# dcvan24/pivot-scheduling

Measured on AMD Instinct MI355X. Metric: task x host placement candidates scored/sec (HBM GB/s % peak) at 1/2/4/8 MI355X, higher is better.
Workload: dtype f64; 1 GPU; synthetic 1000000 hosts x 10000 ready tasks per round, 20 zones, cost_aware best-fit, one independent scenario per GPU; scenarios_per_gpu=1, tasks_per_round=10000, zones=20, policy=ca_bf, parallelism=scenario-sharded x1 (no data-path collective)

## Files before the change

pivot-scheduling_amd/csrc/pvt_zwalk.hip:

```cpp
#include <hip/hip_runtime.h>
#include <stdint.h>

#include "pivot_place.h"
#include "pvt_device.h"
#include "pvt_kernels.h"
#include "pvt_zwin_dev.h"

namespace pvt {

constexpr int ZW_THREADS = 256;
constexpr int ZW_WAVES = ZW_THREADS / 64;
constexpr int ZW_SCAN = 8;
constexpr int ZW_MINB = ZW_MIN_PARTS;
constexpr int ZW_PR = 8;
constexpr double ZW_BIG = 0x1p500;

#ifndef PVT_ZW_UNROLL
#define PVT_ZW_UNROLL 8
#endif
#ifndef PVT_ZW_CF
#define PVT_ZW_CF 0
#endif
constexpr int ZW_UNROLL = PVT_ZW_UNROLL;
constexpr int ZW_SB = 64;
template <int WM>
struct ZwalkLDS {
  double wa[4][WM];
  int32_t wid[WM];
  int32_t wz[WM];
  uint64_t zm[WM / 64];
  double csum[ZMAX * ZMAX], bsum[ZMAX * ZMAX];
  int32_t cnt[ZW_SCAN][ZW_WAVES];
  double red[ZW_WAVES][12];
  double smin[ZW_SB][4];
  double lg[128][4];
  int32_t lgid[128];
  int32_t rwho[64], rstart[64];
  uint64_t sbits[CHAIN_MAX / 64];
  uint32_t amask[ZMAX];
  uint32_t umask;
  int32_t nwin, bail;
  int32_t touch[WM / 64];
};

__device__ __forceinline__ double nan_max(double a, double b) {
  return (a != a || b <= a) ? a : b;
}
__device__ __forceinline__ double wave_nmax_d(double v) {
  return wave_reduce_d(v, [](double a, double b) { return nan_max(a, b); });
}

__global__ __launch_bounds__(256) void host_min_kernel(const double* avail, int H, int lo, int hi,
                                                       double* part) {
  __shared__ double red[4][4];
  const int tid = threadIdx.x, lane = tid & 63, wave = tid >> 6;
  double m[4] = {DINF, DINF, DINF, DINF};
  for (int h = lo + blockIdx.x * 256 + tid; h < hi; h += gridDim.x * 256)
#pragma unroll
    for (int r = 0; r < 4; r++) m[r] = fmin(m[r], avail[(size_t)r * H + h]);
#pragma unroll
  for (int r = 0; r < 4; r++) {
    m[r] = wave_min_d(m[r]);
    if (lane == 0) red[wave][r] = m[r];
  }
  __syncthreads();
  if (tid < 4) {
    double v = red[0][tid];
    for (int w = 1; w < 4; w++) v = fmin(v, red[w][tid]);
    part[blockIdx.x * 4 + tid] = v;
  }
}

template <int N> struct IntC { static constexpr int value = N; };

constexpr int ZW_CAP = 128;
__device__ __forceinline__ int lowbit_exp(double v) {
  const uint64_t b = (uint64_t)__double_as_longlong(v);
  const uint64_t m = b & ((1ull << 52) - 1);
  const int e = (int)((b >> 52) & 0x7ff);
  if (e == 0) return m ? -1074 + __builtin_ctzll(m) : 4096;
  return (e - 1075) + __builtin_ctzll(m | (1ull << 52));
}
__device__ __forceinline__ int high_exp(double v) {
  return (int)(((uint64_t)__double_as_longlong(v) >> 52) & 0x7ff) - 1023;
}
template <bool STRICT>
__device__ __forceinline__ int copies_cf(double x, double d, bool& sure) {
  if (__double_as_longlong(d) == 0) return ZW_CAP;
  const double q = x * __builtin_amdgcn_rcp(d);
  double kf = STRICT ? __builtin_ceil(q) - 1.0 : __builtin_floor(q);
  kf = __builtin_fmin(kf, (double)ZW_CAP);
  const double e0 = __builtin_fma(-kf, d, x), e1 = __builtin_fma(-(kf + 1.0), d, x);
  const double big = __builtin_fabs(x) + (kf + 1.0) * d;
  const bool nice = high_exp(big) + 2 <= min(lowbit_exp(x), lowbit_exp(d)) + 53;
  const double err = nice ? 0.0 : (kf + 2.0) * 0x1p-52 * (big + d);
  const bool fit0 = STRICT ? (e0 > err) : (e0 >= err && (nice || e0 > err));
  const bool out1 = kf >= (double)ZW_CAP || (STRICT ? (e1 <= -err && (nice || e1 < -err)) : (e1 < -err));
  sure = sure && kf >= 1.0 && fit0 && out1 && (q == q);
  return (int)kf;
}

#define UNI(c) (__builtin_amdgcn_readfirstlane((int)(c)) != 0)

template <bool STRICT>
__device__ __forceinline__ bool fit_res(double m) { return STRICT ? (m > 0.0) : (m >= 0.0); }

__device__ __forceinline__ void wave_lds_sync() {
  __atomic_signal_fence(__ATOMIC_SEQ_CST);
  __builtin_amdgcn_s_waitcnt(0xc07f);
  __atomic_signal_fence(__ATOMIC_SEQ_CST);
}

template <int WM = ZW_M>
__device__ __forceinline__ void compact_zone_window(const int32_t* zone, int Z, uint32_t U,
                                                    int h_lo, int h_hi, int32_t* wid, int32_t* wz,
                                                    int32_t (*cnt)[ZW_WAVES], int32_t* nwin) {
  compact_zone_window_t<WM, ZW_THREADS, ZW_SCAN>(zone, Z, U, h_lo, h_hi, wid, wz, cnt, nwin);
}

#ifdef PVT_STAMPS
__device__ __forceinline__ uint64_t zstamp() {
  uint64_t t;
  __builtin_amdgcn_sched_barrier(0);
  asm volatile("s_memtime %0\n\ts_waitcnt lgkmcnt(0)" : "=s"(t)::"memory");
  __builtin_amdgcn_sched_barrier(0);
  return t;
}
#endif

template <bool KEYED, bool STRICT, bool FF = false, int WM = ZW_M, bool FAST = false>
__global__ __launch_bounds__(ZW_THREADS) void zwalk_kernel(ZwalkArgs A) {
  static_assert(!FF || (!KEYED && STRICT), "FF: chain mode, strict fit");
  static_assert(WM == ZW_M || !KEYED, "keyed / ordered / sharded windows: ZW_M hosts");
  __shared__ ZwalkLDS<WM> S;
#ifdef PVT_STAMPS
  const uint64_t t_start = zstamp();
  uint64_t n_chunks = 0, n_switch = 0, n_bulk = 0, n_runs = 0;
  uint64_t st_search = 0, st_p1 = 0, st_p2 = 0, n_probe = 0, n_iter = 0, st_batch = 0, n_single = 0;
  uint64_t st_setup = 0, st_loop = 0, st_who = 0, st_rep = 0;
  uint64_t n_cf = 0;
#endif
  const int b = blockIdx.x, tid = threadIdx.x, lane = tid & 63, wave = tid >> 6;
  const bool tabm = !KEYED && A.tab.nch > 0;
  const int base = KEYED ? 0 : tabm ? A.tab.coff[b] : A.coff[b];
  const int nt = KEYED ? A.knt : tabm ? A.tab.coff[b + 1] - A.tab.coff[b] : A.coff[b + 1] - base;
  const int32_t* gcmap = KEYED ? nullptr : A.cmap + base;
  auto cmap_at = [&](int i) -> int { return gcmap[i]; };
  const bool segm = !KEYED && (tabm || A.cseg);
  int32_t* status = A.status + 2 * b;
  const int Z = A.Z, H = A.H;
  auto report = [&](int s0, int s1) {
    status[0] = s0; status[1] = s1;
    if (!KEYED && A.hstat) { A.hstat[2 * b] = s0; A.hstat[2 * b + 1] = s1; }
  };

  auto publish_map = [&]() {
    if (tabm) {
      int32_t* wmap = const_cast<int32_t*>(A.cmap) + base;
      for (int k = A.tab.csoff[b]; k < A.tab.csoff[b + 1]; k++) {
        const int sg = A.tab.csegid[k], c0 = A.tab.seg_cstart[sg], o0 = A.tab.seg_off[sg];
        const int len = A.tab.seg_off[sg + 1] - o0;
        for (int i = tid; i < len; i += ZW_THREADS) wmap[c0 + i] = o0 + i;
      }
      if (b == 0) {
        const int ns = A.tab.nseg, nc = A.tab.nch;
        for (int i = tid; i <= ns; i += ZW_THREADS) {
          A.tab.o_seg_off[i] = A.tab.seg_off[i];
          if (i < ns) { A.tab.o_seg_chain[i] = A.tab.seg_chain[i]; A.tab.o_seg_cstart[i] = A.tab.seg_cstart[i]; }
        }
        for (int i = tid; i <= nc; i += ZW_THREADS) A.tab.o_coff[i] = A.tab.coff[i];
      }
    }
  };
  double mn[4];
  uint32_t U;
  int nwin;
#ifdef PVT_STAMPS
  uint64_t t_load, t_cert, t_win, t_cap;
#endif
  if constexpr (FAST) {
    static_assert(!KEYED && !FF && WM == ZW_M && ZW_M == 4 * ZW_THREADS, "fast prologue: best-fit chains");
    static_assert(ZW_ENT <= 64 && ZW_ENT <= ZW_SB, "entries: a lane each, in rwho / rstart / lg");
    const int j = min((int)A.cert.cwin[b], ZMAX - 1);
    const ZoneWindow* const zw = &A.zpre->w[j];
    const int ZZ = Z * Z;
    double cs[4], bs[4], ha[4];
#pragma unroll
    for (int u = 0; u < 4; u++) {
      const int i = tid + u * ZW_THREADS;
      cs[u] = i < ZZ ? A.csum[i] : 0.0;
      bs[u] = i < ZZ ? A.bsum[i] : 0.0;
    }
#pragma unroll
    for (int r = 0; r < 4; r++) ha[r] = A.hmin[tid * 4 + r];
    const uint32_t zu = A.zpre->U[j];
    const int zn = zw->n, zbad = zw->bad;
    int32_t wi[4], wzv[4];
    double wv[4][4];
#pragma unroll
    for (int u = 0; u < 4; u++) {
      const int p = tid + u * ZW_THREADS;
      wi[u] = zw->id[p];
      wzv[u] = zw->z[p];
#pragma unroll
      for (int r = 0; r < 4; r++) wv[u][r] = zw->a[r][p];
    }
    const int k0 = A.tab.csoff[b], k1 = A.tab.csoff[b + 1];
    double mxv = -DINF;
    bool badv = false;
    for (int k = k0 + wave; k < k1; k += ZW_WAVES) {
      const int sg = A.tab.csegid[k], c0 = A.tab.seg_cstart[sg];
      const int len = A.tab.seg_off[sg + 1] - A.tab.seg_off[sg];
      const GroupCert* const gc = A.cert.rec + min((int)A.cert.seg_grp[sg], GCOMPACT_MAX - 1);
      const int ne = (len + 63) >> 6, e = A.cert.seg_ent[sg] + lane;
      const bool on = lane < ne && lane < GC_SUB && e < ZW_ENT;
      double sm[4];
#pragma unroll
      for (int r = 0; r < 4; r++) sm[r] = on ? gc->smin[lane][r] : DINF;
      const double gm = lane < 4 ? gc->mx[lane] : -DINF;
      badv |= gc->bad != 0 || gc->n != len;
      mxv = fmax(mxv, gm);
      if (on) {
#pragma unroll
        for (int r = 0; r < 4; r++) S.lg[e][r] = sm[r];
        S.rstart[e] = c0 + 64 * lane;
        S.rwho[e] = c0 + min(64 * lane + 64, len);
      }
    }
    publish_map();
#pragma unroll
    for (int u = 0; u < 4; u++) {
      const int i = tid + u * ZW_THREADS;
      if (i < ZZ) { S.csum[i] = cs[u]; S.bsum[i] = bs[u]; }
    }
    if (tid < CHAIN_MAX / 64) S.sbits[tid] = 0;
    if (tid < WM / 64) S.touch[tid] = 0;
    if (tid < ZW_SB) {
#pragma unroll
      for (int r = 0; r < 4; r++) S.smin[tid][r] = -DINF;
    }
    nwin = min(zn, ZW_M);
#pragma unroll
    for (int u = 0; u < 4; u++) {
      const int p = tid + u * ZW_THREADS;
      if (p < nwin) {
        S.wid[p] = wi[u];
        S.wz[p] = wzv[u];
#pragma unroll
        for (int r = 0; r < 4; r++) S.wa[r][p] = wv[u][r];
      }
    }
#pragma unroll
    for (int r = 0; r < 4; r++) ha[r] = wave_min_d(ha[r]);
    const bool wbadv = __ballot(badv) != 0;
    if (lane < 4) S.red[wave][lane] = mxv;
    if (lane == 0) {
#pragma unroll
      for (int r = 0; r < 4; r++) S.red[wave][8 + r] = ha[r];
      S.cnt[0][wave] = wbadv ? 1 : 0;
    }
#ifdef PVT_STAMPS
    t_load = zstamp();
#endif
    __syncthreads();
    if (tid < Z) {
      uint32_t m = 0;
      for (int z = 0; z < Z; z++) m |= (S.csum[tid * Z + z] == 0.0) ? (1u << z) : 0u;
      S.amask[tid] = m;
    }
    for (int k = k0 + tid; k < k1; k += ZW_THREADS) {
      const int p = A.tab.seg_cstart[A.tab.csegid[k]];
      if (p > 0 && p < CHAIN_MAX) atomicOr(&S.sbits[p >> 6], 1ull << (p & 63));
    }
    double mx[4];
    bool bad = false;
#pragma unroll
    for (int w = 0; w < ZW_WAVES; w++) bad |= S.cnt[0][w] != 0;
#pragma unroll
    for (int r = 0; r < 4; r++) {
      mx[r] = fmax(fmax(S.red[0][r], S.red[1][r]), fmax(S.red[2][r], S.red[3][r]));
      ha[r] = fmin(fmin(S.red[0][8 + r], S.red[1][8 + r]), fmin(S.red[2][8 + r], S.red[3][8 + r]));
    }
    const int ne = min((int)A.cert.cent[b], ZW_ENT);
    {
      double v = lane < ne ? S.lg[lane][wave] : DINF;
#pragma unroll
      for (int off = 1; off < 64; off <<= 1) v = fmin(v, __shfl_down(v, off));
      if (lane < ne) {
        const int q = (S.rstart[lane] + 63) >> 6;
        if (q * 64 < S.rwho[lane] && q < ZW_SB) S.smin[q][wave] = v;
      }
      if (lane == 0) S.red[0][4 + wave] = v;
    }
    bool sep = false;
#pragma unroll
    for (int r = 0; r < 4; r++) sep |= (ha[r] - mx[r] >= 0x1p-288);
    U = zu;
    const bool cover = zu != 0 && (A.cert.cu[b] & ~zu) == 0;
    const bool stop = bad || !sep || nt <= 0 || nt > CHAIN_MAX || !cover || zbad != 0 || nwin <= 0;
#ifdef PVT_STAMPS
    t_cert = t_win = t_cap = zstamp();
#endif
    __syncthreads();
    if (tid == 0) {
      int cert = stop ? 0 : ZW_CERT_FAST;
#pragma unroll
      for (int r = 0; r < 4; r++) {
        const double mnr = S.red[0][4 + r];
        cert |= ((mx[r] <= 0.0 && mnr >= 0.0) ? (1 << r) : 0) | ((ha[r] >= 0x1p-287) ? (16 << r) : 0);
      }
      if (A.hcert) A.hcert[b] = cert;
      if (stop) report(0, nt <= 0 ? 0 : 1);
    }
    if (A.cmax && tid < 4) A.cmax[b * 4 + tid] = mx[tid];
    if (stop) return;
  } else {
    static_assert(ZMAX * ZMAX <= 4 * ZW_THREADS && ZW_MINB == ZW_THREADS, "prologue loads");
    const int ZZ = KEYED ? 0 : Z * Z;
    double cs[4], bs[4];
#pragma unroll
    for (int u = 0; u < 4; u++) {
      const int i = tid + u * ZW_THREADS;
      cs[u] = i < ZZ ? A.csum[i] : 0.0;
      bs[u] = i < ZZ ? A.bsum[i] : 0.0;
    }
    double ha[4] = {FF ? -DINF : DINF, FF ? -DINF : DINF, FF ? -DINF : DINF, FF ? -DINF : DINF};
    if (!KEYED) {
#pragma unroll
      for (int r = 0; r < 4; r++) {
        const double x = A.hmin[tid * 4 + r];
        ha[r] = FF ? nan_max(ha[r], x) : fmin(ha[r], x);
      }
    }
    publish_map();
    int wv[ZW_PR];
    if (tabm) {
      const int k0 = A.tab.csoff[b], k1 = A.tab.csoff[b + 1];
#pragma unroll
      for (int u = 0; u < ZW_PR; u++) {
        const int i = u * ZW_THREADS + tid;
        int v = -1;
        for (int k = k0; k < k1; k++) {
          const int sg = A.tab.csegid[k], c0 = A.tab.seg_cstart[sg];
          if (i >= c0) v = A.tab.seg_off[sg] + (i - c0);
        }
        wv[u] = i < nt ? v : -1;
      }
    } else {
#pragma unroll
      for (int u = 0; u < ZW_PR; u++) {
        const int i = u * ZW_THREADS + tid;
        wv[u] = i < nt ? (KEYED ? i : gcmap[i]) : -1;
      }
    }
    const int sg0 = tabm ? A.tab.csoff[b] : (!KEYED && A.cseg) ? A.csoff[b] : 0;
    const int sg1 = tabm ? A.tab.csoff[b + 1] : (!KEYED && A.cseg) ? A.csoff[b + 1] : 0;
    const uint32_t zpu = (!KEYED && WM == ZW_M && A.zpre && lane < Z) ? A.zpre->U[lane] : 0u;

#pragma unroll
    for (int u = 0; u < 4; u++) {
      const int i = tid + u * ZW_THREADS;
      if (i < ZZ) { S.csum[i] = cs[u]; S.bsum[i] = bs[u]; }
    }
    if (tid == 0) { S.umask = 0; S.nwin = 0; S.bail = 0; }
    if (tid < CHAIN_MAX / 64) S.sbits[tid] = 0;
    if (tid < WM / 64) S.touch[tid] = 0;
#ifdef PVT_STAMPS
    t_load = zstamp();
#endif
    __syncthreads();
    if (!KEYED && tid < Z) {
      uint32_t m = 0;
      for (int z = 0; z < Z; z++) m |= (S.csum[tid * Z + z] == 0.0) ? (1u << z) : 0u;
      S.amask[tid] = m;
    }
    if (tabm) {
      for (int k = sg0 + tid; k < sg1; k += ZW_THREADS) {
        const int p = A.tab.seg_cstart[A.tab.csegid[k]];
        if (p > 0 && p < CHAIN_MAX) atomicOr(&S.sbits[p >> 6], 1ull << (p & 63));
      }
    } else {
      for (int k = sg0 + tid; k < sg1; k += ZW_THREADS) {
        const int p = A.cseg[k];
        if (p > 0 && p < CHAIN_MAX) atomicOr(&S.sbits[p >> 6], 1ull << (p & 63));
      }
    }

    uint32_t abits = 0;
    double mx[4] = {-DINF, -DINF, -DINF, -DINF};
    mn[0] = mn[1] = mn[2] = mn[3] = DINF;
    bool bad = false;
    for (int i0 = 0; i0 < nt; i0 += ZW_PR * ZW_THREADS) {
      int av[ZW_PR], wn[ZW_PR];
      double dv[ZW_PR][4];
#pragma unroll
      for (int u = 0; u < ZW_PR; u++) {
        const int w = max(wv[u], 0);
        av[u] = A.anc[w];
#pragma unroll
        for (int r = 0; r < 4; r++) dv[u][r] = A.dem[(size_t)w * 4 + r];
      }
#pragma unroll
      for (int u = 0; u < ZW_PR; u++) {
        const int i = i0 + ZW_PR * ZW_THREADS + u * ZW_THREADS + tid;
        wn[u] = i < nt ? (KEYED ? i : cmap_at(i)) : -1;
      }
#pragma unroll
      for (int u = 0; u < ZW_PR; u++) {
        const bool ok = wv[u] >= 0;
        double bm[4];
#pragma unroll
        for (int r = 0; r < 4; r++) bm[r] = ok ? dv[u][r] : DINF;
        if (ok) {
          const int a = av[u];
          if (a < 0 || a >= Z) {
            bad = true;
          } else {
            abits |= 1u << a;
#pragma unroll
            for (int r = 0; r < 4; r++) {
              bad |= !(__builtin_fabs(dv[u][r]) <= ZW_BIG);
              mx[r] = fmax(mx[r], dv[u][r]);
              mn[r] = fmin(mn[r], dv[u][r]);
            }
          }
        }
        const int blk = (i0 + u * ZW_THREADS) / 64 + wave;
        if (blk < ZW_SB - 1 && blk * 64 < nt) {
#pragma unroll
          for (int r = 0; r < 4; r++) bm[r] = wave_min_d(bm[r]);
          if (lane == 0) {
#pragma unroll
            for (int r = 0; r < 4; r++) S.smin[blk][r] = bm[r];
          }
        }
      }
#pragma unroll
      for (int u = 0; u < ZW_PR; u++) wv[u] = wn[u];
    }
    __syncthreads();
    uint32_t um = 0;
    if (!KEYED)
      for (uint32_t m = abits; m; m &= m - 1) um |= S.amask[__builtin_ctz(m)];
#pragma unroll
    for (int r = 0; r < 4; r++) {
      mx[r] = wave_max_d(mx[r]);
      mn[r] = wave_min_d(mn[r]);
      ha[r] = FF ? wave_nmax_d(ha[r]) : wave_min_d(ha[r]);
    }
    if (lane == 0) {
#pragma unroll
      for (int r = 0; r < 4; r++) { S.red[wave][r] = mx[r]; S.red[wave][4 + r] = mn[r]; S.red[wave][8 + r] = ha[r]; }
    }
    if (bad) S.bail = 1;
    if (um) atomicOr(&S.umask, um);
    __syncthreads();
#ifdef PVT_STAMPS
    t_cert = zstamp();
#endif
#pragma unroll
    for (int r = 0; r < 4; r++) {
      for (int w = 1; w < ZW_WAVES; w++) {
        mx[r] = fmax(mx[r], S.red[w][r]);
        mn[r] = fmin(mn[r], S.red[w][4 + r]);
        ha[r] = FF ? nan_max(ha[r], S.red[w][8 + r]) : fmin(ha[r], S.red[w][8 + r]);
      }
      mx[r] = fmax(mx[r], S.red[0][r]);
      mn[r] = fmin(mn[r], S.red[0][4 + r]);
      ha[r] = FF ? nan_max(ha[r], S.red[0][8 + r]) : fmin(ha[r], S.red[0][8 + r]);
    }
    if (!KEYED && A.cmax && tid < 4) A.cmax[b * 4 + tid] = mx[tid];
    if (!KEYED && A.hcert && tid == 0) {
      int cert = 0;
      if (!FF) {
#pragma unroll
        for (int r = 0; r < 4; r++)
          cert |= ((mx[r] <= 0.0 && mn[r] >= 0.0) ? (1 << r) : 0) | ((ha[r] >= 0x1p-287) ? (16 << r) : 0);
      }
      A.hcert[b] = cert;
    }
    bool sep = KEYED;
    if (FF) {
      sep = true;
#pragma unroll
      for (int r = 0; r < 4; r++) sep &= (ha[r] <= 0x1p298) && (mn[r] >= 0.0);
    } else {
#pragma unroll
      for (int r = 0; r < 4; r++) sep |= (ha[r] - mx[r] >= 0x1p-288);
    }
    U = S.umask;
    if (S.bail || !sep || nt <= 0 || (!KEYED && nt > CHAIN_MAX)) {
      if (tid == 0) report(0, (KEYED || nt <= 0) ? 0 : 1);
      return;
    }
    const FrontierSlot* pw = A.pwin ? A.pwin + (KEYED ? 0 : b) : nullptr;
    const ZoneWindow* zw = nullptr;
    if (!KEYED && WM == ZW_M && !pw && A.zpre && U != 0) {
      const uint64_t cover = __ballot(zpu != 0 && (U & ~zpu) == 0);
      if (cover) {
        const int j = __builtin_ctzll(cover);
        zw = &A.zpre->w[j];
        U = (uint32_t)__builtin_amdgcn_readlane((int)zpu, j);
      }
    }
    if (pw) {
      const int nw = min(pw->n, ZW_M);
      for (int p = tid; p < nw; p += ZW_THREADS) {
        const int32_t h = pw->id[p];
        S.wid[p] = h;
        S.wz[p] = KEYED ? 0 : A.zone[h];
      }
      if (tid == 0) S.nwin = nw;
      __syncthreads();
    } else if (zw) {
      const int nw = min(zw->n, ZW_M);
      for (int p = tid; p < nw; p += ZW_THREADS) { S.wid[p] = zw->id[p]; S.wz[p] = zw->z[p]; }
      if (tid == 0) S.nwin = nw;
      __syncthreads();
    } else if (KEYED) {
      const int nw = min(A.kn_dev ? *A.kn_dev : A.kn, ZW_M);
      for (int p = tid; p < nw; p += ZW_THREADS) { S.wid[p] = A.lo + A.kperm[p]; S.wz[p] = 0; }
      if (tid == 0) S.nwin = nw;
      __syncthreads();
    } else {
      compact_zone_window<WM>(A.zone, Z, U, 0, H, S.wid, S.wz, S.cnt, &S.nwin);
    }
    nwin = S.nwin;
#ifdef PVT_STAMPS
    t_win = zstamp();
#endif
    bool wbad = false;
    ZwUndo* const ud = (!KEYED && A.undo) ? A.undo + b : nullptr;
    if (ud && tid == 0) ud->count = nwin;
    static_assert(WM <= ZW_MBIG, "ZwUndo holds every window");
    static_assert(WM % (4 * ZW_THREADS) == 0, "window capacities: four hosts per thread per pass");
    for (int p0 = 0; p0 < WM && p0 < nwin; p0 += 4 * ZW_THREADS) {
      double v[4][4];
#pragma unroll
      for (int u = 0; u < 4; u++) {
        const int p = p0 + u * ZW_THREADS + tid;
        const int h = p < nwin ? S.wid[p] : 0;
#pragma unroll
        for (int r = 0; r < 4; r++)
          v[u][r] = p >= nwin ? 0.0 : (pw ? pw->a[r][p] : zw ? zw->a[r][p] : A.avail[(size_t)r * H + h]);
      }
#pragma unroll
      for (int u = 0; u < 4; u++) {
        const int p = p0 + u * ZW_THREADS + tid;
        if (p < nwin) {
#pragma unroll
          for (int r = 0; r < 4; r++) {
            wbad |= !(__builtin_fabs(v[u][r]) <= ZW_BIG);
            S.wa[r][p] = v[u][r];
          }
          if (ud) {
            ud->id[p] = S.wid[p];
#pragma unroll
            for (int r = 0; r < 4; r++) ud->a[r][p] = v[u][r];
          }
        }
      }
    }
    if (wbad) S.bail = 1;
    __syncthreads();
#ifdef PVT_STAMPS
    t_cap = zstamp();
#endif
    if (S.bail || nwin == 0) {
      if (tid == 0) report(0, KEYED ? 0 : 1);
      return;
    }
    const int nsb = min((nt + 63) >> 6, ZW_SB);
    for (int blk = ZW_SB - 1 + wave; blk < nsb; blk += ZW_WAVES) {
      const int i1 = blk == ZW_SB - 1 ? nt : min(nt, blk * 64 + 64);
      double bm[4] = {DINF, DINF, DINF, DINF};
      for (int i = blk * 64 + lane; i < i1; i += 64) {
        const int w = KEYED ? i : cmap_at(i);
#pragma unroll
        for (int r = 0; r < 4; r++) bm[r] = fmin(bm[r], A.dem[(size_t)w * 4 + r]);
      }
#pragma unroll
      for (int r = 0; r < 4; r++) bm[r] = wave_min_d(bm[r]);
      if (lane == 0) {
#pragma unroll
        for (int r = 0; r < 4; r++) S.smin[blk][r] = bm[r];
      }
    }
    __syncthreads();
    static_assert(ZW_SB == 64 && ZW_WAVES == 4, "suffix minima: one wave per dimension, a lane per batch");
    {
      double v = lane < nsb ? S.smin[lane][wave] : DINF;
#pragma unroll
      for (int off = 1; off < 64; off <<= 1) v = fmin(v, __shfl_down(v, off));
      if (lane < nsb) S.smin[lane][wave] = v;
    }
    __syncthreads();
  }
  if (wave != 0) return;
#ifdef PVT_STAMPS
  const uint64_t t_walk = zstamp();
#endif

  const int nch = (nwin + 63) >> 6;
  int p0 = 0;
  int cur = -1;
  int done = 0;
  bool failed = false, exhausted = false;
  double ra0, ra1, ra2, ra3;
  int32_t rid;
  uint64_t rzm = 0, rvalid = 0;
  bool dirty = false;
  auto load_chunk = [&](int c) {
    const int p = c * 64 + lane;
    const int q = min(p, nwin - 1);
    ra0 = S.wa[0][q]; ra1 = S.wa[1][q]; ra2 = S.wa[2][q]; ra3 = S.wa[3][q];
    rid = S.wid[q];
    rvalid = __ballot(p < nwin);
    dirty = false;
    __builtin_amdgcn_s_waitcnt(0xc07f);
  };
  auto store_chunk = [&](int c) {
    const int p = c * 64 + lane;
    if (dirty && p < nwin) { S.wa[0][p] = ra0; S.wa[1][p] = ra1; S.wa[2][p] = ra2; S.wa[3][p] = ra3; }
    dirty = false;
  };
  double rb0 = 0.0, rb1 = 0.0, rb2 = 0.0, rb3 = 0.0;
  int32_t bid = 0;
  uint64_t bzm = 0, bvalid = 0;
  bool bdirty = false;
  int pb = -1;
  auto load_b = [&](int c) {
    bdirty = false;
    if (c >= nch) { pb = -1; bvalid = 0; bzm = 0; return; }
    pb = c;
    const int p = c * 64 + lane;
    const int q = min(p, nwin - 1);
    rb0 = S.wa[0][q]; rb1 = S.wa[1][q]; rb2 = S.wa[2][q]; rb3 = S.wa[3][q];
    bid = S.wid[q];
    bvalid = __ballot(p < nwin);
    bzm = cur >= 0 ? rfl_u64(S.zm[c]) : 0;
    __builtin_amdgcn_s_waitcnt(0xc07f);
  };
  auto store_b = [&]() {
    const int p = pb * 64 + lane;
    if (bdirty && pb >= 0 && p < nwin) { S.wa[0][p] = rb0; S.wa[1][p] = rb1; S.wa[2][p] = rb2; S.wa[3][p] = rb3; }
    bdirty = false;
  };
  auto run_bulk = [&](auto cft, double& c0, double& c1, double& c2, double& c3, int32_t cid, double d0,
                      double d1, double d2, double d3, uint64_t m0, int R, int k) -> int {
#ifdef PVT_STAMPS
    const uint64_t tA = zstamp();
#endif
    if (!(d0 >= 0.0 && d1 >= 0.0 && d2 >= 0.0 && d3 >= 0.0)) R = 1;
    const bool on1 = __builtin_amdgcn_inverse_ballot_w64(m0);
    const bool two = __double_as_longlong(d2) == 0 && __double_as_longlong(d3) == 0;
    R = __builtin_amdgcn_readfirstlane(R);
    int cnt = 0;
#ifdef PVT_STAMPS
    const uint64_t tA1 = zstamp();
    st_setup += tA1 - tA;
#endif
    bool cf = false;
#if PVT_ZW_CF
    if (decltype(cft)::value && R >= 2) {
      bool sure = true;
      int k = ZW_CAP;
      if (on1) {
        k = min(copies_cf<STRICT>(c0, d0, sure), copies_cf<STRICT>(c1, d1, sure));
        if (!two) k = min(k, min(copies_cf<STRICT>(c2, d2, sure), copies_cf<STRICT>(c3, d3, sure)));
      }
      const bool bad = on1 && !sure;
      const uint64_t ub = __ballot(bad);
      const int kc = on1 && sure ? k : 0;
      const int inc = wave_incl_scan_dpp(kc);
      const int first_bad = ub ? __builtin_ctzll(ub) : 64;
      const int before_bad = first_bad == 0 ? 0 : __builtin_amdgcn_readlane(inc, first_bad - 1);
      cf = ub == 0 || before_bad >= R;
      if (cf) cnt = (lane < first_bad) ? kc : 0;
#ifdef PVT_STAMPS
      n_cf += cf;
#endif
    }
#endif
    if (!cf) {
      double x0 = on1 ? c0 : -DINF, x1 = on1 ? c1 : -DINF, x2 = on1 ? c2 : -DINF, x3 = on1 ? c3 : -DINF;
      int t = 0;
      auto pass1 = [&](auto dims) {
        constexpr int D = decltype(dims)::value;
        int u = __builtin_ctzll(m0), fb = 0;
        for (;;) {
          t = __builtin_amdgcn_readfirstlane(t);
          u = __builtin_amdgcn_readfirstlane(u);
          fb = __builtin_amdgcn_readfirstlane(fb);
          bool f = false;
#pragma unroll
          for (int j = 1; j <= ZW_UNROLL; j++) {
            x0 -= d0; x1 -= d1;
            if (D == 4) { x2 -= d2; x3 -= d3; }
            f = fit_res<STRICT>(D == 4 ? fmin(fmin(x0, x1), fmin(x2, x3)) : fmin(x0, x1));
            cnt = f ? t + j : cnt;
          }
          t += ZW_UNROLL;
          const uint64_t an = __ballot(f);
          if (UNI(an == 0)) break;
          const int un = __builtin_ctzll(an);
          if (un != u) {
            u = un;
            fb = __builtin_amdgcn_readlane(wave_incl_scan_dpp(cnt), u - 1);
          }
          if (UNI(fb + t >= R)) break;
        }
      };
      if (two) pass1(IntC<2>{});
      else pass1(IntC<4>{});
#ifdef PVT_STAMPS
      n_iter += t;
#endif
    }
#ifdef PVT_STAMPS
    st_loop += zstamp() - tA1;
#endif
    const int incl = wave_incl_scan_dpp(cnt);
    const int pre = incl - cnt;
    const int asg = max(0, min(cnt, R - pre));
    const int covered = min(R, __builtin_amdgcn_readlane(incl, 63));
#ifdef PVT_STAMPS
    const uint64_t tB = zstamp();
    st_p1 += tB - tA;
#endif
    S.rstart[lane] = 0;
    if (asg > 0) { S.rstart[pre] = 1; S.rwho[pre] = cid; }
    wave_lds_sync();
    const uint64_t starts = __ballot(S.rstart[lane] != 0);
    const uint64_t upto = starts & (lane == 63 ? ~0ull : ((2ull << lane) - 1ull));
    const int32_t who = upto ? S.rwho[63 - __builtin_clzll(upto)] : 0;
    const int amax = wave_max_i32(asg);
    if (lane < covered) S.lgid[k + lane] = who;
#ifdef PVT_STAMPS
    const uint64_t tC = zstamp();
    st_who += tC - tB;
#endif
    if (two) {
      for (int m = 0; m < amax; m += 4) {
#pragma unroll
        for (int u = 0; u < 4; u++) {
          const double o = m + u < asg ? -1.0 : -0.0;
          c0 = __builtin_fma(o, d0, c0);
          c1 = __builtin_fma(o, d1, c1);
        }
      }
    } else {
      for (int m = 0; m < amax; m += 4) {
#pragma unroll
        for (int u = 0; u < 4; u++) {
          const double o = m + u < asg ? -1.0 : -0.0;
          c0 = __builtin_fma(o, d0, c0);
          c1 = __builtin_fma(o, d1, c1);
          c2 = __builtin_fma(o, d2, c2);
          c3 = __builtin_fma(o, d3, c3);
        }
      }
    }
#ifdef PVT_STAMPS
    st_rep += zstamp() - tC;
#endif
    if (asg > 0) {
      const int q = k + pre + asg - 1;
      S.lg[q][0] = c0; S.lg[q][1] = c1; S.lg[q][2] = c2; S.lg[q][3] = c3;
    }
#ifdef PVT_STAMPS
    st_p2 += zstamp() - tB;
#endif
    return covered;
  };
  load_chunk(0);
  load_b(1);
  auto task_at = [&](int i) { return i < nt ? (KEYED ? i : cmap_at(i)) : 0; };
  int nw = task_at(lane);
  double nd0 = A.dem[(size_t)nw * 4 + 0], nd1 = A.dem[(size_t)nw * 4 + 1];
  double nd2 = A.dem[(size_t)nw * 4 + 2], nd3 = A.dem[(size_t)nw * 4 + 3];
  int nanc = A.anc[nw], ncal = A.ord[nw];
  int nw1 = task_at(64 + lane);
  int carry = 0;
  for (int i0 = 0; UNI(i0 < nt && !failed); i0 += 64) {
#ifdef PVT_STAMPS
    uint64_t tb0 = zstamp();
#endif
#pragma unroll
    for (int r = 0; r < 4; r++) mn[r] = S.smin[min(i0 >> 6, ZW_SB - 1)][r];
    const int tw = nw;
    const double td[4] = {nd0, nd1, nd2, nd3};
    const int tanc = nanc;
    const int tcal = ncal;
    if (i0 + 64 < nt) {
      nw = nw1;
      nd0 = A.dem[(size_t)nw * 4 + 0]; nd1 = A.dem[(size_t)nw * 4 + 1];
      nd2 = A.dem[(size_t)nw * 4 + 2]; nd3 = A.dem[(size_t)nw * 4 + 3];
      nanc = A.anc[nw]; ncal = A.ord[nw];
      nw1 = task_at(i0 + 128 + lane);
    }
    const int kn = min(64, nt - i0);
    bool uni = __ballot(lane < kn && tanc != cur) == 0;
    uint64_t E;
    {
      bool same = lane > 0 && lane < kn;
#pragma unroll
      for (int r = 0; r < 4; r++)
        same &= __double_as_longlong(__shfl_up(td[r], 1)) == __double_as_longlong(td[r]);
      E = __ballot(same);
      if (segm) E &= ~rfl_u64(S.sbits[i0 >> 6]);
    }
    int extc = -1;
    auto ext_len = [&]() -> int {
      if (extc < 0) {
        extc = 0;
        if (kn == 64 && i0 + 64 < nt && uni) {
          const int kn2 = min(64, nt - i0 - 64);
          const double l0 = readlane_d(td[0], 63), l1 = readlane_d(td[1], 63);
          const double l2 = readlane_d(td[2], 63), l3 = readlane_d(td[3], 63);
          bool eq = lane < kn2 && readlane_i(tanc, 63) == nanc &&
                    __double_as_longlong(nd0) == __double_as_longlong(l0) &&
                    __double_as_longlong(nd1) == __double_as_longlong(l1) &&
                    __double_as_longlong(nd2) == __double_as_longlong(l2) &&
                    __double_as_longlong(nd3) == __double_as_longlong(l3);
          if (segm) eq = eq && !((rfl_u64(S.sbits[(i0 >> 6) + 1]) >> lane) & 1ull);
          const uint64_t m = __ballot(eq);
          extc = m == ~0ull ? 64 : __builtin_ctzll(~m);
        }
        extc = __builtin_amdgcn_readfirstlane(extc);
      }
      return extc;
    };
    auto run_len = [&](int k) {
      int r = k < 63 ? min(kn - k, 1 + __builtin_ctzll(~(E >> (k + 1)))) : 1;
      if (k + r == 64) r = min(64, r + ext_len());
      return r;
    };
    auto run_step = [&](int k) -> int {
#ifdef PVT_STAMPS
      const uint64_t t0 = zstamp();
#define ZW_SEARCH_DONE() (st_search += zstamp() - t0)
#else
#define ZW_SEARCH_DONE() ((void)0)
#endif
      const double d0 = readlane_d(td[0], k), d1 = readlane_d(td[1], k);
      const double d2 = readlane_d(td[2], k), d3 = readlane_d(td[3], k);
      const int R = run_len(k);
      for (;;) {
        const double n0 = ra0 - d0, n1 = ra1 - d1, n2 = ra2 - d2, n3 = ra3 - d3;
        uint64_t fm = __ballot(fit_res<STRICT>(fmin(fmin(n0, n1), fmin(n2, n3)))) & rvalid;
        if (FF) fm &= rzm;
        if (!FF && UNI((fm & ~rzm) != 0)) return 0;
        if (UNI(fm != 0)) {
          dirty = true;
          ZW_SEARCH_DONE();
          return run_bulk(IntC<0>{}, ra0, ra1, ra2, ra3, rid, d0, d1, d2, d3, fm, R, k);
        }
        if (__ballot(((rvalid >> lane) & 1ull) && fits<STRICT>(ra0, ra1, ra2, ra3, mn[0], mn[1], mn[2], mn[3])))
          break;
        if (p0 + 1 >= nch) return 0;
        store_b();
        store_chunk(p0);
        ++p0;
        rzm = rfl_u64(S.zm[p0]);
        load_chunk(p0);
        load_b(p0 + 1);
      }
      if (pb >= 0) {
        const double q0 = rb0 - d0, q1 = rb1 - d1, q2 = rb2 - d2, q3 = rb3 - d3;
        uint64_t fb = __ballot(fit_res<STRICT>(fmin(fmin(q0, q1), fmin(q2, q3)))) & bvalid;
        if (FF) fb &= bzm;
        if (!FF && UNI((fb & ~bzm) != 0)) return 0;
        if (UNI(fb != 0)) {
          bdirty = true;
          ZW_SEARCH_DONE();
          return run_bulk(IntC<0>{}, rb0, rb1, rb2, rb3, bid, d0, d1, d2, d3, fb, R, k);
        }
      }
      for (int c = (pb >= 0 ? pb : p0) + 1; c < nch; c++) {
        const int p = c * 64 + lane;
        const int q = min(p, nwin - 1);
        double x0 = S.wa[0][q], x1 = S.wa[1][q], x2 = S.wa[2][q], x3 = S.wa[3][q];
        const int32_t xid = S.wid[q];
        const uint64_t xzm = rfl_u64(S.zm[c]);
#ifdef PVT_STAMPS
        n_probe++;
#endif
        uint64_t fm = __ballot(p < nwin && fit_res<STRICT>(fmin(fmin(x0 - d0, x1 - d1),
                                                                fmin(x2 - d2, x3 - d3))));
        if (FF) fm &= xzm;
        if (!FF && UNI((fm & ~xzm) != 0)) return 0;
        if (UNI(fm != 0)) {
          ZW_SEARCH_DONE();
          const int got = run_bulk(IntC<0>{}, x0, x1, x2, x3, xid, d0, d1, d2, d3, fm, R, k);
          if (p < nwin) { S.wa[0][p] = x0; S.wa[1][p] = x1; S.wa[2][p] = x2; S.wa[3][p] = x3; }
          if (!KEYED && lane == 0) S.touch[c] = 1;
          return got;
        }
      }
      ZW_SEARCH_DONE();
      return 0;
    };
#undef ZW_SEARCH_DONE
#ifdef PVT_STAMPS
    st_batch += zstamp() - tb0;
#endif
    int k = carry;
    if (carry) {
      wave_lds_sync();
      if (lane < carry) {
#pragma unroll
        for (int r = 0; r < 4; r++) S.lg[lane][r] = S.lg[64 + lane][r];
        S.lgid[lane] = S.lgid[64 + lane];
      }
      wave_lds_sync();
    }
    while (UNI(k < kn)) {
      k = __builtin_amdgcn_readfirstlane(k);
      p0 = __builtin_amdgcn_readfirstlane(p0);
      pb = __builtin_amdgcn_readfirstlane(pb);
      done = __builtin_amdgcn_readfirstlane(done);
      rzm = rfl_u64(rzm);
      bzm = rfl_u64(bzm);
      if (uni) {
        for (; k < kn;) {
          k = __builtin_amdgcn_readfirstlane(k);
          const double d0 = readlane_d(td[0], k), d1 = readlane_d(td[1], k);
          const double d2 = readlane_d(td[2], k), d3 = readlane_d(td[3], k);
          const double n0 = ra0 - d0, n1 = ra1 - d1, n2 = ra2 - d2, n3 = ra3 - d3;
          const uint64_t fm0 = __ballot(fit_res<STRICT>(fmin(fmin(n0, n1), fmin(n2, n3)))) & rvalid;
          const uint64_t m0 = fm0 & rzm;
          if (UNI(m0 == 0 || (!FF && (fm0 & ~rzm) != 0))) break;
          const int R = run_len(k);
          if (UNI(R >= 2)) {
            const int c = run_bulk(IntC<1>{}, ra0, ra1, ra2, ra3, rid, d0, d1, d2, d3, m0, R, k);
            k += c;
            done += c;
            dirty = true;
#ifdef PVT_STAMPS
            n_chunks += c;
            n_bulk += c;
            n_runs++;
#endif
            continue;
          }
          const bool win = __builtin_amdgcn_inverse_ballot_w64(m0 & (0ull - m0));
          ra0 = win ? n0 : ra0; ra1 = win ? n1 : ra1; ra2 = win ? n2 : ra2; ra3 = win ? n3 : ra3;
          if (win) {
            S.lg[k][0] = n0; S.lg[k][1] = n1; S.lg[k][2] = n2; S.lg[k][3] = n3;
            S.lgid[k] = rid;
          }
          dirty = true;
#ifdef PVT_STAMPS
          n_chunks++;
          n_single++;
#endif
          done++;
          k++;
        }
        if (UNI(k >= kn)) break;
        const int got = run_step(k);
        if (UNI(got > 0)) {
          k += got;
          done += got;
#ifdef PVT_STAMPS
          n_chunks += got;
          n_bulk += got;
          n_runs++;
#endif
          continue;
        }
      }
      const double d0 = readlane_d(td[0], k), d1 = readlane_d(td[1], k);
      const double d2 = readlane_d(td[2], k), d3 = readlane_d(td[3], k);
      const int a = uni ? cur : readlane_i(tanc, k);
      if (a != cur) {
        bool ok = true;
        if (!KEYED && lane < Z) {
          const double c = S.csum[a * Z + lane], bw = S.bsum[a * Z + lane];
          if (c == 0.0) ok = bw > 0.0;
          else if (FF || !((U >> lane) & 1u)) ok = (c >= 0x1p-300) && (bw > 0.0) && (bw <= 0x1p300);
        }
        if (__ballot(!ok)) { failed = true; break; }
        const uint32_t am = KEYED ? ~0u : S.amask[a];
        for (int c = 0; c < nch; c++) {
          const int p = c * 64 + lane;
          const uint64_t m = __ballot(p < nwin && (KEYED || ((am >> S.wz[min(p, nwin - 1)]) & 1u)));
          if (lane == 0) S.zm[c] = m;
          if (c == p0) rzm = m;
          if (c == pb) bzm = m;
        }
        cur = a;
        uni = __ballot(lane >= k && lane < kn && tanc != cur) == 0;
        __builtin_amdgcn_s_waitcnt(0xc07f);
#ifdef PVT_STAMPS
        n_switch++;
#endif
      }
      auto zero_exact = [&](bool f, bool k0, double a0, double a1, double a2, double a3, int q) {
        if (FF) return k0;
        if (__builtin_expect(__ballot(f && !k0) != 0, 0)) {
          if (f && !k0) {
            const int z = S.wz[q];
            const double s2 = norm2_seq(a0 - d0, a1 - d1, a2 - d2, a3 - d3);
            const double sc = (S.csum[a * Z + z] * __builtin_sqrt(s2)) / S.bsum[a * Z + z];
            k0 = __double_as_longlong(sc) == 0;
          }
        }
        return k0;
      };
      const double n0 = ra0 - d0, n1 = ra1 - d1, n2 = ra2 - d2, n3 = ra3 - d3;
      const uint64_t fm0 = __ballot(fit_res<STRICT>(fmin(fmin(n0, n1), fmin(n2, n3)))) & rvalid;
      bool found = true;
#ifdef PVT_STAMPS
      n_chunks++;
#endif
      const uint64_t m0 = fm0 & rzm;
      if (__builtin_expect(m0 != 0 && (FF || (fm0 & ~rzm) == 0), 1)) {
        const bool win = __builtin_amdgcn_inverse_ballot_w64(m0 & (0ull - m0));
        ra0 = win ? n0 : ra0; ra1 = win ? n1 : ra1; ra2 = win ? n2 : ra2; ra3 = win ? n3 : ra3;
        if (win) {
          S.lg[k][0] = n0; S.lg[k][1] = n1; S.lg[k][2] = n2; S.lg[k][3] = n3;
          S.lgid[k] = rid;
        }
        dirty = true;
      } else {
        bool inb = false;
        if (fm0 == 0 && pb >= 0) {
          const double q0 = rb0 - d0, q1 = rb1 - d1, q2 = rb2 - d2, q3 = rb3 - d3;
          const uint64_t fb = __ballot(fit_res<STRICT>(fmin(fmin(q0, q1), fmin(q2, q3)))) & bvalid;
          const uint64_t mb = fb & bzm;
          if (mb != 0 && (FF || (fb & ~bzm) == 0)) {
            const bool win = __builtin_amdgcn_inverse_ballot_w64(mb & (0ull - mb));
            rb0 = win ? q0 : rb0; rb1 = win ? q1 : rb1; rb2 = win ? q2 : rb2; rb3 = win ? q3 : rb3;
            if (win) {
              S.lg[k][0] = q0; S.lg[k][1] = q1; S.lg[k][2] = q2; S.lg[k][3] = q3;
              S.lgid[k] = bid;
            }
            bdirty = true;
            inb = true;
          }
        }
        if (!inb) {
          found = false;
          store_b();
          double g0 = n0, g1 = n1, g2 = n2, g3 = n3;
          uint64_t fm = fm0, m = fm0 & rzm;
#ifdef PVT_STAMPS
          for (int pass = 0;; pass++) {
            n_chunks += pass > 0;
#else
          for (;;) {
#endif
            if (fm & ~rzm)
              m = __ballot(zero_exact((fm >> lane) & 1ull, (rzm >> lane) & 1ull, ra0, ra1, ra2,
                                      ra3, min(p0 * 64 + lane, nwin - 1))) & fm;
            if (m) {
              const bool win = lane == __builtin_ctzll(m);
              ra0 = win ? g0 : ra0; ra1 = win ? g1 : ra1; ra2 = win ? g2 : ra2; ra3 = win ? g3 : ra3;
              if (win) {
                S.lg[k][0] = g0; S.lg[k][1] = g1; S.lg[k][2] = g2; S.lg[k][3] = g3;
                S.lgid[k] = rid;
              }
              dirty = true;
              found = true;
              break;
            }
            if (__ballot(((rvalid >> lane) & 1ull) && fits<STRICT>(ra0, ra1, ra2, ra3, mn[0], mn[1], mn[2], mn[3])))
              break;
            store_chunk(p0);
            if (++p0 >= nch) break;
            rzm = rfl_u64(S.zm[p0]);
            load_chunk(p0);
            g0 = ra0 - d0; g1 = ra1 - d1; g2 = ra2 - d2; g3 = ra3 - d3;
            fm = __ballot(fit_res<STRICT>(fmin(fmin(g0, g1), fmin(g2, g3)))) & rvalid;
            m = fm & rzm;
          }
          if (!found && p0 < nch) {
            store_chunk(p0);
            for (int c = p0 + 1; c < nch; c++) {
#ifdef PVT_STAMPS
              n_chunks++;
#endif
              const int p = c * 64 + lane;
              const int q = min(p, nwin - 1);
              const double a0 = S.wa[0][q], a1 = S.wa[1][q], a2 = S.wa[2][q], a3 = S.wa[3][q];
              const int32_t id = S.wid[q];
              const uint64_t zm = rfl_u64(S.zm[c]);
              const bool f = p < nwin && fits<STRICT>(a0, a1, a2, a3, d0, d1, d2, d3);
              const bool k0 = zero_exact(f, (zm >> lane) & 1ull, a0, a1, a2, a3, q);
              const uint64_t mc = __ballot(f && k0);
              if (mc) {
                if (lane == __builtin_ctzll(mc)) {
                  const double c0 = a0 - d0, c1 = a1 - d1, c2 = a2 - d2, c3 = a3 - d3;
                  S.wa[0][q] = c0; S.wa[1][q] = c1; S.wa[2][q] = c2; S.wa[3][q] = c3;
                  S.lg[k][0] = c0; S.lg[k][1] = c1; S.lg[k][2] = c2; S.lg[k][3] = c3;
                  S.lgid[k] = id;
                  if (!KEYED) S.touch[c] = 1;
                }
                found = true;
                break;
              }
            }
          }
          wave_lds_sync();
          load_b(p0 + 1);
        }
      }
      if (UNI(!found)) {
        failed = true;
        exhausted = nwin >= WM;
        break;
      }
      done++;
      k++;
    }
#ifdef PVT_STAMPS
    tb0 = zstamp();
#endif
    if (lane < k) {
      WinRec& e = A.wlog[tw];
      const int32_t id = S.lgid[lane];
      e.s = 0.0;
      e.id = id;
      e.a[0] = S.lg[lane][0]; e.a[1] = S.lg[lane][1]; e.a[2] = S.lg[lane][2]; e.a[3] = S.lg[lane][3];
      A.placement[tcal] = id;
    }
    carry = __builtin_amdgcn_readfirstlane(k > kn ? k - kn : 0);
#ifdef PVT_STAMPS
    st_batch += zstamp() - tb0;
#endif
  }
  if (KEYED) {
    store_chunk(p0);
    store_b();
    wave_lds_sync();
    for (int p = lane; p < nwin; p += 64) {
      const int h = S.wid[p];
#pragma unroll
      for (int r = 0; r < 4; r++) A.wb[(size_t)r * H + h] = S.wa[r][p];
    }
  }
  if (!KEYED && A.undo && !failed && done == nt) {
    store_chunk(p0);
    store_b();
    wave_lds_sync();
    const int top = max(p0, pb);
    for (int c = 0; c < nch; c++) {
      if (c > top && !S.touch[c]) continue;
      const int p = c * 64 + lane;
      if (p < nwin) {
        const int h = S.wid[p];
#pragma unroll
        for (int r = 0; r < 4; r++) A.wb[(size_t)r * H + h] = S.wa[r][p];
      }
    }
  }
  if (lane == 0) report(done, (failed && !KEYED) ? (exhausted ? 2 : 1) : 0);
#ifdef PVT_STAMPS
  if (lane == 0 && A.stamps) {
    const uint64_t t_end = zstamp();
    atomicAdd((unsigned long long*)&A.stamps[0], (unsigned long long)(t_walk - t_start));
    atomicAdd((unsigned long long*)&A.stamps[1], (unsigned long long)(t_end - t_walk));
    atomicAdd((unsigned long long*)&A.stamps[2], (unsigned long long)n_chunks);
    atomicAdd((unsigned long long*)&A.stamps[3], (unsigned long long)done);
    atomicAdd((unsigned long long*)&A.stamps[4], (unsigned long long)n_switch);
    atomicAdd((unsigned long long*)&A.stamps[5], (unsigned long long)n_bulk);
    atomicAdd((unsigned long long*)&A.stamps[6], (unsigned long long)n_runs);
    atomicAdd((unsigned long long*)&A.stamps[7], (unsigned long long)st_search);
    atomicAdd((unsigned long long*)&A.stamps[8], (unsigned long long)st_p1);
    atomicAdd((unsigned long long*)&A.stamps[9], (unsigned long long)st_p2);
    atomicAdd((unsigned long long*)&A.stamps[10], (unsigned long long)n_probe);
    atomicAdd((unsigned long long*)&A.stamps[11], (unsigned long long)n_iter);
    atomicAdd((unsigned long long*)&A.stamps[12], (unsigned long long)st_batch);
    atomicAdd((unsigned long long*)&A.stamps[13], (unsigned long long)n_single);
    atomicAdd((unsigned long long*)&A.stamps[20], (unsigned long long)(t_cert - t_start));
    atomicAdd((unsigned long long*)&A.stamps[21], (unsigned long long)(t_win - t_cert));
    atomicAdd((unsigned long long*)&A.stamps[22], (unsigned long long)(t_cap - t_win));
    atomicAdd((unsigned long long*)&A.stamps[23], (unsigned long long)(t_walk - t_cap));
    atomicAdd((unsigned long long*)&A.stamps[24], (unsigned long long)st_setup);
    atomicAdd((unsigned long long*)&A.stamps[25], (unsigned long long)st_loop);
    atomicAdd((unsigned long long*)&A.stamps[26], (unsigned long long)st_who);
    atomicAdd((unsigned long long*)&A.stamps[27], (unsigned long long)st_rep);
    atomicAdd((unsigned long long*)&A.stamps[28], (unsigned long long)n_cf);
    atomicAdd((unsigned long long*)&A.stamps[29], (unsigned long long)(t_load - t_start));
  }
#endif
}

void launch_host_min(const double* avail, int H, int lo, int hi, double* part, hipStream_t st) {
  PVT_LAUNCH(host_min_kernel, dim3(ZW_MINB), dim3(256), 0, st, avail, H, lo, hi, part);
}

void launch_zwalk(const ZwalkArgs& a, int nchains, hipStream_t st) {
  if (a.cert.fast && a.tab.nch > 0 && a.zpre && !a.pwin)
    PVT_LAUNCH((zwalk_kernel<false, false, false, ZW_M, true>), dim3(nchains), dim3(ZW_THREADS), 0, st, a);
  else
    PVT_LAUNCH((zwalk_kernel<false, false>), dim3(nchains), dim3(ZW_THREADS), 0, st, a);
}
void launch_zwalk_big(const ZwalkArgs& a, int nchains, hipStream_t st) {
  PVT_LAUNCH((zwalk_kernel<false, false, false, ZW_MBIG>), dim3(nchains), dim3(ZW_THREADS), 0, st, a);
}
void launch_zwalk_ff(const ZwalkArgs& a, int nchains, hipStream_t st) {
  PVT_LAUNCH((zwalk_kernel<false, true, true>), dim3(nchains), dim3(ZW_THREADS), 0, st, a);
}

__global__ __launch_bounds__(256) void host_absmax_kernel(const double* avail, int H, int lo, int hi,
                                                          double* part) {
  __shared__ double red[4][4];
  const int tid = threadIdx.x, lane = tid & 63, wave = tid >> 6;
  double m[4] = {0.0, 0.0, 0.0, 0.0};
  for (int h = lo + blockIdx.x * 256 + tid; h < hi; h += gridDim.x * 256)
#pragma unroll
    for (int r = 0; r < 4; r++) {
      m[r] = nan_max(m[r], __builtin_fabs(avail[(size_t)r * H + h]));
    }
#pragma unroll
  for (int r = 0; r < 4; r++) {
    m[r] = wave_nmax_d(m[r]);
    if (lane == 0) red[wave][r] = m[r];
  }
  __syncthreads();
  if (tid < 4) {
    double v = red[0][tid];
    for (int w = 1; w < 4; w++) v = nan_max(v, red[w][tid]);
    part[blockIdx.x * 4 + tid] = v;
  }
}
void launch_host_absmax(const double* avail, int H, int lo, int hi, double* part, hipStream_t st) {
  PVT_LAUNCH(host_absmax_kernel, dim3(ZW_MINB), dim3(256), 0, st, avail, H, lo, hi, part);
}
void launch_zwalk_keyed(const ZwalkArgs& a, bool strict, hipStream_t st) {
  if (strict) PVT_LAUNCH((zwalk_kernel<true, true>), dim3(1), dim3(ZW_THREADS), 0, st, a);
  else PVT_LAUNCH((zwalk_kernel<true, false>), dim3(1), dim3(ZW_THREADS), 0, st, a);
}

__global__ __launch_bounds__(1024) void dem_min_kernel(const double* dem, int n, double* out) {
  __shared__ double red[16][4];
  const int tid = threadIdx.x, lane = tid & 63, wave = tid >> 6;
  double m[4] = {DINF, DINF, DINF, DINF};
  for (int i = tid; i < n; i += 1024)
#pragma unroll
    for (int r = 0; r < 4; r++) m[r] = fmin(m[r], dem[(size_t)i * 4 + r]);
#pragma unroll
  for (int r = 0; r < 4; r++) {
    m[r] = wave_min_d(m[r]);
    if (lane == 0) red[wave][r] = m[r];
  }
  __syncthreads();
  if (tid < 4) {
    double v = red[0][tid];
    for (int w = 1; w < 16; w++) v = fmin(v, red[w][tid]);
    out[tid] = v;
  }
}
__global__ void alive_flags_kernel(const double* avail, int H, int lo, int hs, const double* dmin,
                                   int strict, uint8_t* flags) {
  const int h = lo + blockIdx.x * blockDim.x + threadIdx.x;
  if (h >= hs) return;
  const double a0 = avail[h], a1 = avail[(size_t)H + h], a2 = avail[2 * (size_t)H + h],
               a3 = avail[3 * (size_t)H + h];
  flags[h - lo] = strict ? fits<true>(a0, a1, a2, a3, dmin[0], dmin[1], dmin[2], dmin[3])
                    : fits<false>(a0, a1, a2, a3, dmin[0], dmin[1], dmin[2], dmin[3]);
}
void launch_alive_flags(const double* avail, int H, int lo, int hs, const double* dem, int n,
                        int strict, double* dmin, uint8_t* flags, hipStream_t st) {
  PVT_LAUNCH(dem_min_kernel, dim3(1), dim3(1024), 0, st, dem, n, dmin);
  if (hs <= lo) return;
  PVT_LAUNCH(alive_flags_kernel, dim3((hs - lo + 255) / 256), dim3(256), 0, st, avail, H,
                     lo, hs, dmin, strict, flags);
}


__global__ __launch_bounds__(ZW_THREADS) void zwin_build_kernel(ZwinArgs A) {
  __shared__ uint32_t amask[ZMAX];
  __shared__ uint32_t umask;
  __shared__ int32_t cnt[ZW_SCAN][ZW_WAVES];
  __shared__ int32_t nwin;
  const int b = blockIdx.x, tid = threadIdx.x, Z = A.Z;
  FrontierSlot* out = A.out + b;
  if (tid == 0) { umask = 0; nwin = 0; }
  if (tid < Z) {
    uint32_t m = 0;
    for (int z = 0; z < Z; z++) m |= (A.csum[tid * Z + z] == 0.0) ? (1u << z) : 0u;
    amask[tid] = m;
  }
  __syncthreads();
  uint32_t um = 0;
  for (int i = A.coff[b] + tid; i < A.coff[b + 1]; i += ZW_THREADS) {
    const int a = A.anc[A.cmap[i]];
    if (a >= 0 && a < Z) um |= amask[a];
  }
  if (um) atomicOr(&umask, um);
  __syncthreads();
  compact_zone_window(A.zone, Z, umask, A.lo, A.hi, out->id, nullptr, cnt, &nwin);
  const int n = nwin;
  for (int p = tid; p < n; p += ZW_THREADS) {
    const int h = out->id[p];
#pragma unroll
    for (int r = 0; r < 4; r++) out->a[r][p] = A.avail[(size_t)r * A.H + h];
  }
  if (tid == 0) { out->n = n; out->total = n; }
}

__global__ __launch_bounds__(256) void zwin_gather_kernel(const double* avail, int H, int lo,
                                                          const int32_t* perm, const int32_t* count,
                                                          FrontierSlot* out) {
  const int c = *count, n = min(c, ZW_M);
  for (int p = threadIdx.x; p < n; p += 256) {
    const int h = lo + perm[p];
    out->id[p] = h;
#pragma unroll
    for (int r = 0; r < 4; r++) out->a[r][p] = avail[(size_t)r * H + h];
  }
  if (threadIdx.x == 0) { out->n = n; out->total = c; }
}

__global__ __launch_bounds__(256) void zwin_merge_kernel(const uint8_t* pkgs, int64_t pkg_bytes,
                                                         int world, int nslots, FrontierSlot* out,
                                                         double* hmin) {
  __shared__ int32_t off[PVT_SHARD_MAX_WORLD + 1];
  const int b = blockIdx.x, tid = threadIdx.x;
  auto hdr = [&](int k) { return reinterpret_cast<const FrontierHdr*>(pkgs + (size_t)k * pkg_bytes); };
  if (b == nslots) {
    for (int i = tid; hmin && i < ZW_MIN_PARTS * 4; i += 256) {
      double m = DINF;
      for (int k = 0; k < world; k++) m = fmin(m, (&hdr(k)->hmin[0][0])[i]);
      (&hmin[0])[i] = m;
    }
    return;
  }
  auto slot = [&](int k) { return reinterpret_cast<const FrontierSlot*>(hdr(k) + 1) + b; };
  if (tid == 0) {
    int o = 0, tot = 0;
    for (int k = 0; k < world; k++) { off[k] = o; o += slot(k)->n; tot += slot(k)->total; }
    off[world] = o;
    out[b].n = min(o, ZW_M);
    out[b].total = tot;
  }
  __syncthreads();
  for (int k = 0; k < world && off[k] < ZW_M; k++) {
    const FrontierSlot* s = slot(k);
    const int n = min(s->n, ZW_M - off[k]);
    for (int p = tid; p < n; p += 256) {
      const int q = off[k] + p;
      out[b].id[q] = s->id[p];
#pragma unroll
      for (int r = 0; r < 4; r++) out[b].a[r][q] = s->a[r][p];
    }
  }
}

void launch_zwin_build(const ZwinArgs& a, int nchains, hipStream_t st) {
  PVT_LAUNCH(zwin_build_kernel, dim3(nchains), dim3(ZW_THREADS), 0, st, a);
}
void launch_zwin_gather(const double* avail, int H, int lo, const int32_t* perm,
                        const int32_t* count, FrontierSlot* out, hipStream_t st) {
  PVT_LAUNCH(zwin_gather_kernel, dim3(1), dim3(256), 0, st, avail, H, lo, perm, count, out);
}
void launch_zwin_merge(const uint8_t* pkgs, int64_t pkg_bytes, int world, int nslots,
                       FrontierSlot* out, double* hmin, hipStream_t st) {
  PVT_LAUNCH(zwin_merge_kernel, dim3(nslots + 1), dim3(256), 0, st, pkgs, pkg_bytes, world,
                     nslots, out, hmin);
}

}
```

Before: 55290 billion candidates/s.

## Defer per-batch win-log writes and resolve run owners lazily via sentinel fill

Result: faster. 57150 billion candidates/s (median of 6 runs) (+3.4%).

```diff
diff --git a/pivot-scheduling_amd/csrc/pvt_zwalk.hip b/pivot-scheduling_amd/csrc/pvt_zwalk.hip
--- a/pivot-scheduling_amd/csrc/pvt_zwalk.hip
+++ b/pivot-scheduling_amd/csrc/pvt_zwalk.hip
@@ -23,6 +23,7 @@
 #endif
 constexpr int ZW_UNROLL = PVT_ZW_UNROLL;
 constexpr int ZW_SB = 64;
+constexpr int32_t ZW_SAME = -1;
 template <int WM>
 struct ZwalkLDS {
   double wa[4][WM];
@@ -728,14 +729,8 @@
     const uint64_t tB = zstamp();
     st_p1 += tB - tA;
 #endif
-    S.rstart[lane] = 0;
-    if (asg > 0) { S.rstart[pre] = 1; S.rwho[pre] = cid; }
-    wave_lds_sync();
-    const uint64_t starts = __ballot(S.rstart[lane] != 0);
-    const uint64_t upto = starts & (lane == 63 ? ~0ull : ((2ull << lane) - 1ull));
-    const int32_t who = upto ? S.rwho[63 - __builtin_clzll(upto)] : 0;
+    if (asg > 0) S.lgid[k + pre] = cid;
     const int amax = wave_max_i32(asg);
-    if (lane < covered) S.lgid[k + lane] = who;
 #ifdef PVT_STAMPS
     const uint64_t tC = zstamp();
     st_who += tC - tB;
@@ -782,6 +777,26 @@
   int nanc = A.anc[nw], ncal = A.ord[nw];
   int nw1 = task_at(64 + lane);
   int carry = 0;
+  int fk = 0, ftw = 0, fcal = 0;
+  int32_t fprev = 0;
+  S.lgid[lane] = ZW_SAME;
+  S.lgid[64 + lane] = ZW_SAME;
+  auto flush_log = [&]() {
+    if (UNI(fk > 0)) {
+      const int32_t raw = S.lgid[lane];
+      const uint64_t upto = __ballot(raw != ZW_SAME) & (lane == 63 ? ~0ull : ((2ull << lane) - 1ull));
+      const int32_t from = __shfl(raw, upto ? 63 - __builtin_clzll(upto) : 0);
+      const int32_t id = upto ? from : fprev;
+      fprev = __builtin_amdgcn_readlane(id, 63);
+      if (lane < fk) {
+        WinRec& e = A.wlog[ftw];
+        e.s = 0.0;
+        e.id = id;
+        e.a[0] = S.lg[lane][0]; e.a[1] = S.lg[lane][1]; e.a[2] = S.lg[lane][2]; e.a[3] = S.lg[lane][3];
+        A.placement[fcal] = id;
+      }
+    }
+  };
   for (int i0 = 0; UNI(i0 < nt && !failed); i0 += 64) {
 #ifdef PVT_STAMPS
     uint64_t tb0 = zstamp();
@@ -792,6 +807,10 @@
     const double td[4] = {nd0, nd1, nd2, nd3};
     const int tanc = nanc;
     const int tcal = ncal;
+    __atomic_signal_fence(__ATOMIC_SEQ_CST);
+    __builtin_amdgcn_s_waitcnt(0x0f70);
+    __atomic_signal_fence(__ATOMIC_SEQ_CST);
+    flush_log();
     if (i0 + 64 < nt) {
       nw = nw1;
       nd0 = A.dem[(size_t)nw * 4 + 0]; nd1 = A.dem[(size_t)nw * 4 + 1];
@@ -906,13 +925,15 @@
     st_batch += zstamp() - tb0;
 #endif
     int k = carry;
-    if (carry) {
+    {
       wave_lds_sync();
+      const int32_t cid = lane < carry ? S.lgid[64 + lane] : ZW_SAME;
       if (lane < carry) {
 #pragma unroll
         for (int r = 0; r < 4; r++) S.lg[lane][r] = S.lg[64 + lane][r];
-        S.lgid[lane] = S.lgid[64 + lane];
-      }
+      }
+      S.lgid[lane] = cid;
+      S.lgid[64 + lane] = ZW_SAME;
       wave_lds_sync();
     }
     while (UNI(k < kn)) {
@@ -1118,19 +1139,15 @@
 #ifdef PVT_STAMPS
     tb0 = zstamp();
 #endif
-    if (lane < k) {
-      WinRec& e = A.wlog[tw];
-      const int32_t id = S.lgid[lane];
-      e.s = 0.0;
-      e.id = id;
-      e.a[0] = S.lg[lane][0]; e.a[1] = S.lg[lane][1]; e.a[2] = S.lg[lane][2]; e.a[3] = S.lg[lane][3];
-      A.placement[tcal] = id;
-    }
+    fk = __builtin_amdgcn_readfirstlane(k);
+    ftw = tw;
+    fcal = tcal;
     carry = __builtin_amdgcn_readfirstlane(k > kn ? k - kn : 0);
 #ifdef PVT_STAMPS
     st_batch += zstamp() - tb0;
 #endif
   }
+  flush_log();
   if (KEYED) {
     store_chunk(p0);
     store_b();
```
